# pdishuck/GAVISUNK

Measured on NVIDIA B200. Metric: ont_read_gbp_per_s_sunk_matched_validated, higher is better.
Workload: dtype u64

## Files before the change

### gavisunk_b200/_lib.py

```python
from __future__ import annotations

import ctypes as C
import os

_HERE = os.path.dirname(os.path.abspath(__file__))
LIB_PATH = os.environ.get("GVS_LIB_PATH") or os.path.join(_HERE, "libgavisunk_b200.so")

u8p, u32p, u64p, i32p, i64p, f64p = (C.POINTER(t) for t in (C.c_uint8, C.c_uint32, C.c_uint64, C.c_int32, C.c_int64, C.c_double))
vp = C.c_void_p

PROTOTYPES = {
    "gvs_create": (vp, [C.c_int, C.c_int]),
    "gvs_destroy": (None, [vp]),
    "gvs_last_error": (C.c_char_p, [vp]),
    "gvs_version": (C.c_char_p, []),
    "gvs_set_stream": (C.c_int, [vp, vp]),
    "gvs_sync": (C.c_int, [vp]),
    "gvs_set_profiling": (C.c_int, [vp, C.c_int]),
    "gvs_stage_ms": (C.c_int, [vp, C.c_int, C.POINTER(C.c_float)]),
    "gvs_launch_count": (C.c_uint64, [vp]),
    "gvs_host_alloc": (C.c_int, [C.c_uint64, C.POINTER(vp)]),
    "gvs_host_free": (None, [vp]),
    "gvs_db_load_loc": (C.c_int, [vp, vp, C.c_uint64, vp, vp, vp, vp, C.c_uint64, C.c_uint32]),
    "gvs_db_build": (C.c_int, [vp, vp, vp, C.c_uint32, C.c_int]),
# ... 16 lines not shown
    "gvs_best_get": (C.c_int, [vp, vp, vp, vp, vp]),
    "gvs_filter_best": (C.c_int, [vp, vp, u64p]),
    "gvs_contigs_set": (C.c_int, [vp, vp, vp, C.c_uint32]),
    "gvs_group_hist":(C.c_int, [vp, C.c_int, C.POINTER(vp)]),
    "gvs_hist_mode": (C.c_int, [vp, i64p]),
    "gvs_bad_groups": (C.c_int, [vp, i64p, u64p]),
    "gvs_bad_get": (C.c_int, [vp, vp]),
    "gvs_bad_set": (C.c_int, [vp, vp, vp, C.c_uint64, u64p]),
    "gvs_groups_count": (C.c_int, [vp, u64p]),
    "gvs_groups_get": (C.c_int, [vp, vp, vp, vp]),
    "gvs_batches_begin": (C.c_int, [vp]),
    "gvs_batch_stash": (C.c_int, [vp, u64p]),
    "gvs_batches_bind": (C.c_int, [vp, u64p, u64p]),
    "gvs_validate": (C.c_int, [vp, C.c_uint32, u64p]),
    "gvs_pairs_get": (C.c_int, [vp, vp, vp, vp, vp]),
    "gvs_components_local": (C.c_int, [vp, C.POINTER(vp)]),
    "gvs_components_merge_all": (C.c_int, [vp, vp, C.c_uint32, C.c_uint32]),
    "gvs_placements": (C.c_int, [vp, u64p, C.POINTER(vp)]),
    "gvs_placements_get": (C.c_int, [vp, vp, vp, vp, vp, vp, vp]),
    "gvs_support": (C.c_int, [vp, vp, u64p]),
    "gvs_support_get": (C.c_int, [vp, vp, vp, vp, vp]),
    "gvs_spans": (C.c_int, [vp, C.c_uint32, C.c_uint32, u64p, C.POINTER(vp)]),
    "gvs_spans_get": (C.c_int, [vp] * 9),
    "gvs_discordance": (C.c_int, [vp, vp, u64p]),
    "gvs_discordance_get": (C.c_int, [vp] * 7),
    "gvs_intervals": (C.c_int, [vp, u64p]),
    "gvs_intervals_get": (C.c_int, [vp, vp, vp, vp]),
    "gvs_intervals_set": (C.c_int, [vp, vp, vp, vp, C.c_uint64, C.c_uint32]),
    "gvs_gaps": (C.c_int, [vp, vp, u64p, u64p]),
    "gvs_gaps_get": (C.c_int, [vp, vp, vp, vp, vp]),
# ... 74 lines not shown
```

### gavisunk_b200/csrc/common.cuh

```cuda
#pragma once
#include <cuda_runtime.h>
#include <stdint.h>
#include <stdio.h>
#include <string.h>

#include <string>
#include <vector>

#include "../../include/gavisunk_b200.h"

typedef uint8_t u8;
typedef uint16_t u16;
typedef uint32_t u32;
typedef uint64_t u64;
typedef int32_t i32;
typedef int64_t i64;

#define GVS_NSM_DEFAULT 148
#define GVS_TILE_BASES 512
#define GVS_SEG_COUNT 16
#define GVS_SEG_COUNT_PACK 48
#define GVS_SEG_MIN_BYTES (256ull << 20)

struct DevBuf {
  void* p = nullptr;
  size_t cap = 0;
  template <typename T>
  T* as() const { return (T*)p; }
};

struct Rows {
  DevBuf read, pos, contig, start, group, gidx;
  u64 n = 0;
};

struct RecTable {
  DevBuf buf;
// ... 1 lines not shown
  bool ready = false;
  u32* col(u32 t) const { return buf.as<u32>() + t * stride; }
};

struct gvs_ctx {
  int device = 0;
  int k = 20;
  int n_sm = GVS_NSM_DEFAULT;
  cudaStream_t stream = 0;
  std::string err;
  u64 launches = 0;
  bool profiling = false;
  cudaEvent_t ev0[GVS_ST_COUNT], ev1[GVS_ST_COUNT];
  bool ev_valid[GVS_ST_COUNT];
  std::vector<void*> pinned;
  cudaStream_t aux[2] = {nullptr, nullptr};
  bool val_attr_set = false;
  int l2_persist_max = -1, l2_window_max = 0;
  size_t l2_carve_set = 0;
  cudaEvent_t ev_fork = nullptr, ev_join[2] = {nullptr, nullptr};

  bool db_ready = false;
  u64 n_loc = 0, n_groups = 0;
  u32 n_contigs = 0;
  DevBuf loc_kmer, loc_contig, loc_start, loc_group, loc_gidx;
  DevBuf loc_pack;
  DevBuf grp_contig, grp_start;
  u64 grp_gen = 0;
  DevBuf tab_keys, tab_rows, tab_kv;
  u64 tab_slots = 0;
  DevBuf filt;
  u64 filt_words = 0;
  bool filt_fp = false;
  int probe_variant = 0;
  DevBuf filt1;
// ... 140 lines not shown
                      cudaGetErrorString(e__));                                             \
  } while (0)

#define LAUNCH_ON(strm, kern, grid, block, smem, ...)                                       \
  do {                                                                                      \
    kern<<<(grid), (block), (smem), (strm)>>>(__VA_ARGS__);                                 \
    ctx->launches++;                                                                        \
    cudaError_t e__ = cudaGetLastError();                                                   \
    if (e__ != cudaSuccess)                                                                 \
      return gvs_fail(ctx, GVS_E_CUDA, "%s:%d launch %s: %s", __FILE__, __LINE__, #kern,    \
                      cudaGetErrorString(e__));                                             \
  } while (0)

static inline int gvs_fork(gvs_ctx* ctx) {
  if (!ctx->aux[0]) {
    for (int i = 0; i < 2; i++) {
      CK(cudaStreamCreateWithFlags(&ctx->aux[i], cudaStreamNonBlocking));
      CK(cudaEventCreateWithFlags(&ctx->ev_join[i], cudaEventDisableTiming));
    }
    CK(cudaEventCreateWithFlags(&ctx->ev_fork, cudaEventDisableTiming));
  }
  CK(cudaEventRecord(ctx->ev_fork, ctx->stream));
  for (int i = 0; i < 2; i++) CK(cudaStreamWaitEvent(ctx->aux[i], ctx->ev_fork, 0));
  return 0;
}
static inline int gvs_join(gvs_ctx* ctx) {
  for (int i = 0; i < 2; i++) {
    CK(cudaEventRecord(ctx->ev_join[i], ctx->aux[i]));
    CK(cudaStreamWaitEvent(ctx->stream, ctx->ev_join[i], 0));
  }
  return 0;
}

static inline int gvs_reserve(gvs_ctx* ctx, DevBuf& b, size_t bytes) {
  if (bytes == 0) bytes = 16;
  if (b.cap >= bytes) return 0;
  if (b.p) {
    CK(cudaStreamSynchronize(ctx->stream));
    CK(cudaFree(b.p));
    b.p = nullptr;
    b.cap = 0;
  }
// ... 309 lines not shown
```

### gavisunk_b200/csrc/ctx.cu

```cuda
#include "common.cuh"

#include <sched.h>
#include <stdlib.h>

#include <atomic>
#include <chrono>
#include <condition_variable>
#include <mutex>
#include <thread>

extern "C" void gvs_hostpack_range(const uint8_t* ascii, uint64_t n, uint32_t* words, uint64_t w0, uint64_t w1);

struct HostPipe {
  std::vector<std::thread> workers;
  std::mutex mu;
  std::condition_variable cv_job, cv_done;
  u64 gen = 0;
  bool quit = false;
  int running = 0;
  const u8* ascii = nullptr;
  u64 n = 0;
  u32* words = nullptr;
  u64 w_end = 0;
  std::atomic<u64> next{0};
// ... 145 lines not shown
                   &c->seg_orient, &c->rank_of, &c->rank_grp, &c->sup_diff, &c->pl_strand, &c->pl_tmp,
                   &c->sup_depth, &c->sup_gx, &c->sup_cstat, &c->ge_seg_start, &c->ge_cgap, &c->ge_seg, &c->ge_cand, &c->ge_res,
                   &c->jn_seg_start, &c->jn_row_seg, &c->jn_seg_cnt, &c->jn_flags, &c->jn_scr, &c->dc_diff, &c->dc_scr, &c->dc_seg,
                   &c->pl.buf, &c->sup.buf, &c->ge.buf, &c->jn.buf, &c->dc.buf, &c->dc_runs.buf, &c->rh_scratch, &c->rh.buf,
                   &c->rh_run.buf};
  for (DevBuf* b : all) gvs_release(*b);
  release_rows(c->rows);
  release_rows(c->kept);
  release_rows(c->jn_stash);
  release_rows(c->stash);
  gvs_release(c->stash_len);
  for (int i = 0; i < GVS_ST_COUNT; i++) {
    cudaEventDestroy(c->ev0[i]);
    cudaEventDestroy(c->ev1[i]);
  }
  for (int i = 0; i < 2; i++) {
    if (c->aux[i]) {
      cudaStreamSynchronize(c->aux[i]);
      cudaStreamDestroy(c->aux[i]);
    }
    if (c->ev_join[i]) cudaEventDestroy(c->ev_join[i]);
  }
  if (c->ev_fork) cudaEventDestroy(c->ev_fork);
  for (cudaEvent_t e : c->seg_ev) cudaEventDestroy(e);
  if (c->ev_reads_free) cudaEventDestroy(c->ev_reads_free);
  if (c->copy_stream) {
    cudaStreamSynchronize(c->copy_stream);
    cudaStreamDestroy(c->copy_stream);
  }
  if (c->mailbox) cudaFreeHost(c->mailbox);
  delete c;
// ... 283 lines not shown
```

### gavisunk_b200/csrc/validate_reads.cu

```cuda
#include "common.cuh"

#define VCAP_WARP 64
#define VCAP 512
#define VROW_BYTES 80
#define NOV 0xFFFFFFFFu
#define NOT64 0xFFFFFFFFFFFFFFFFull

#define F_MULTI 1u
#define F_GOOD 2u
#define F_PRES 4u

struct VWork {
  u32 *P, *S, *ID, *G;
  u32 *uP, *uS, *uID, *uG;
  u32 *deg, *rep, *label, *csize, *flags;
  u64 *key, *tv, *ct;
};

__device__ __forceinline__ void vwork_carve(VWork& w, u8* base, u32 cap) {
  u64* q = (u64*)base;
  w.key = q; q += cap;
  w.tv = q; q += cap;
  w.ct = q; q += cap;
  u32* p = (u32*)q;
// ... 3 lines not shown
}

__device__ __forceinline__ bool pair_ok(u32 pi, u32 si, u32 pj, u32 sj) {
  u64 ds = si > sj ? si - sj : sj - si;
  u64 dp = pi > pj ? pi - pj : pj - pi;
  return 9 * ds < 10 * dp && 10 * dp < 11 * ds;
}

struct ValParams : SegRows {
  ReadLens len;
  u32 min_len;
  u32* out_id;
  u32* out_gidx;
  u32* seg_cnt;
  u8* orient;
  u32 m_lo, m_hi;
  u8* gscratch;
  u32 big_cap;
  u32* stats;
};

template <int NT, int GROUPS, bool GLOBAL>
__global__ void __launch_bounds__(NT* GROUPS) k_validate(const ValParams V) {
  extern __shared__ __align__(16) u8 smem[];
  __shared__ u32 s_n0[GROUPS], s_n1[GROUPS], s_m[GROUPS], s_kept[GROUPS], s_bestroot[GROUPS], s_flag[GROUPS], s_dup[GROUPS];
  __shared__ u32 s_pmin[GROUPS], s_pmax[GROUPS];
  __shared__ u32 s_up[GROUPS], s_dn[GROUPS];
  __shared__ unsigned long long s_best[GROUPS];
  __shared__ u32 s_wtot[GROUPS][NT / 32];
  const int grp = threadIdx.x / NT;
  const int tid = threadIdx.x % NT;
  auto gsync = [&]() {
    if (NT == 32) __syncwarp(); else __syncthreads();
  };
  VWork w;
  const u32 cap = GLOBAL ? V.big_cap : (NT == 32 ? VCAP_WARP : VCAP);
  if (GLOBAL) vwork_carve(w, V.gscratch + (u64)blockIdx.x * VROW_BYTES * cap, cap);
  else vwork_carve(w, smem + (u64)grp * VROW_BYTES * cap, cap);

  for (u32 s = blockIdx.x * GROUPS + grp; s < V.n_seg; s += gridDim.x * GROUPS) {
    const u32 a = V.seg_start[s], b = V.seg_start[s + 1];
    const u32 mrows = b - a;
    if (mrows <= V.m_lo || mrows > V.m_hi) continue;
    gsync();
    if (tid == 0) { s_m[grp] = 0; s_n0[grp] = 0; s_n1[grp] = 0; s_kept[grp] = 0; s_best[grp] = 0; s_bestroot[grp] = NOV; s_flag[grp] = 0; s_dup[grp] = 0; s_pmin[grp] = 0xFFFFFFFFu; s_pmax[grp] = 0; s_up[grp] = 0; s_dn[grp] = 0; }
    gsync();
    const u32 rd = V.read[a];
    const u32 rlen = V.len(rd);
    const bool skip = rlen < V.min_len || mrows < 2;
    if (!skip) {
      u32 kept_so_far = 0;
      for (u32 base = 0; base < mrows; base += NT) {
        const u32 i = base + tid;
        bool keep = false;
        u32 gi = 0;
        if (i < mrows) {
          gi = V.gidx[a + i];
          keep = !(V.bad && V.bad[gi]);
        }
        const u32 bal = __ballot_sync(0xFFFFFFFFu, keep);
// ... 50 lines not shown
            u32 sj = w.uS[j], pj = w.uP[j];
            rank += (sj < si) | ((sj == si) & (pj < pi));
          }
        }
        w.P[rank] = pi;
        w.S[rank] = si;
        w.ID[rank] = w.uID[i];
        w.G[rank] = w.uG[i];
        w.csize[i] = 0;
        w.tv[i] = NOT64;
        w.ct[i] = NOT64;
      }
    }
    gsync();
    {
      u32 dupl = 0;
      for (u32 i = tid; i + 1 < m; i += NT) dupl |= w.ID[i] >= w.ID[i + 1];
      if (dupl) s_dup[grp] = 1;
    }
    {
      const u32 id0 = w.ID[0];
      u32 any = 0;
      for (u32 i = tid; i < m; i += NT) any |= w.ID[i] != id0;
      if (any) s_flag[grp] = 1;
    }
    gsync();
    if (!s_flag[grp]) {
      if (tid == 0) V.seg_cnt[s] = 0;
      continue;
    }
    {
      u32 pmin = 0xFFFFFFFFu, pmax = 0;
      for (u32 r = tid; r < m; r += NT) {
// ... 112 lines not shown
        w.flags[r] = present ? F_PRES : 0u;
        w.label[r] = present ? (fp != NOV ? fp : r) : NOV;
        w.tv[r] = present ? tmin : NOT64;
        w.ct[r] = NOT64;
      }
      if (tid == 0) s_kept[grp] = orient ? s_n1[grp] : s_n0[grp];
    } else {
      for (u32 r = tid; r < m; r += NT) {
        if (orient) {
          w.deg[r] = w.label[r];
          w.key[r] = w.ct[r];
        }
        w.ct[r] = NOT64;
      }
      gsync();
      for (u32 r = tid; r < m; r += NT) {
        const u32 id = w.ID[r], dr = w.deg[r];
        const u64 kr = w.key[r];
        u32 first = r, multi = 0, good = dr > 0;
        for (u32 q = 0; q < m; q++) {
          u32 same = (w.ID[q] == id);
          u32 dq = w.deg[q];
          first = (same & (q < first)) ? q : first;
          u32 other = same & (q != r) & (dq > 0);
          multi |= other;
          u32 beats = other & ((dq > dr) | ((dq == dr) & (w.key[q] < kr)));
          good &= beats ^ 1u;
        }
        w.rep[r] = first;
        w.flags[r] = ((multi & (dr > 0)) ? F_MULTI : 0u) | (good ? F_GOOD : 0u);
      }
      gsync();
      {
        u32 nk = 0;
        for (u32 r = tid; r < m; r += NT) {
// ... 33 lines not shown
      continue;
    }
    if (tid == 0) { s_n0[grp] = NOV; s_n1[grp] = 0; }
    gsync();
    for (u32 r = tid; r < m; r += NT)
      if (w.flags[r] & F_PRES) atomicMin(&s_n0[grp], w.label[r]);
    gsync();
    {
      const u32 l0 = s_n0[grp];
      u32 differs = 0;
      for (u32 r = tid; r < m; r += NT) differs |= ((w.flags[r] & F_PRES) != 0) & (w.label[r] != l0);
      if (differs) s_n1[grp] = 1;
    }
    gsync();
    const bool in_row_order = !s_dup[grp] && s_n1[grp] == 0;
    for (int round = 0; s_n1[grp] && round < 4096; round++) {
      if (tid == 0) s_flag[grp] = 0;
      gsync();
      u32 changed = 0;
      for (u32 r = tid; r < m; r += NT) {
        const u32 fr = w.flags[r];
        if (!(fr & F_PRES)) continue;
        const u32 pr = w.P[r], sr = w.S[r], idr = w.ID[r];
        u32 lab = w.label[r];
        const u32 lab0 = lab;
        for (u32 q = 0; q < m; q++) {
          u32 pq = w.P[q], sq = w.S[q], idq = w.ID[q], fq = w.flags[q];
          u32 hi = q > r;
          u32 sg = hi ? (pr > pq) : (pq > pr);
          u32 e = pair_ok(pr, sr, pq, sq) & (q != r) & (sg == orient);
          u32 fl = hi ? fr : fq, fh = hi ? fq : fr;
          u32 drop = ((fl & F_MULTI) != 0) & ((fl & F_GOOD) == 0) & (((fh & F_GOOD) == 0) | (idq != idr));
          u32 link = (e & (drop ^ 1u)) | ((idq == idr) & ((fq & F_PRES) != 0));
          u32 lq = w.label[q];
          lab = (link && lq < lab) ? lq : lab;
        }
        if (lab != lab0) {
          w.label[r] = lab;
          changed = 1;
        }
      }
      if (changed) s_flag[grp] = 1;
      gsync();
      if (!s_flag[grp]) break;
      gsync();
    }
    for (u32 r = tid; r < m; r += NT) {
      u32 fr = w.flags[r];
      if (!(fr & F_PRES)) continue;
      const u32 idr = w.ID[r];
      u32 firstp = r;
      if (s_dup[grp])
        for (u32 q = 0; q < r; q++)
          if (w.ID[q] == idr && (w.flags[q] & F_PRES)) { firstp = q; break; }
      if (firstp != r) continue;
      u32 lab = w.label[r];
      atomicAdd(&w.csize[lab], 1u);
      atomicMin((unsigned long long*)&w.ct[lab], (unsigned long long)w.tv[w.rep[r]]);
      w.flags[r] = fr | 8u;
    }
    gsync();
    for (u32 r = tid; r < m; r += NT) {
      if (w.csize[r]) {
        unsigned long long key = ((unsigned long long)w.csize[r] << 42) | ((1ull << 42) - 1 - w.ct[r]);
        atomicMax(&s_best[grp], key);
      }
    }
    gsync();
// ... 20 lines not shown
          total = 0;
          for (int wv = 0; wv < NT / 32; wv++) {
            const u32 c = s_wtot[grp][wv];
            before += wv < (tid >> 5) ? c : 0u;
            total += c;
          }
        }
        if (mem) {
          const u32 rank = done + before + __popc(bal & ((1u << (tid & 31)) - 1));
          V.out_id[a + rank] = w.ID[r];
          V.out_gidx[a + rank] = w.G[r];
        }
        done += total;
        if (NT > 32) gsync();
      }
    } else
    for (u32 r = tid; r < m; r += NT) {
      if ((w.flags[r] & 8u) && w.label[r] == broot) {
        const u64 t = w.tv[w.rep[r]];
        u32 rank = 0;
        for (u32 q = 0; q < m; q++) rank += ((w.flags[q] & 8u) != 0) & (w.label[q] == broot) & (w.tv[w.rep[q]] < t);
        V.out_id[a + rank] = w.ID[r];
        V.out_gidx[a + rank] = w.G[r];
      }
    }
    if (tid == 0) {
      V.seg_cnt[s] = w.csize[broot];
      V.orient[s] = (u8)orient;
    }
  }
}

__global__ void __launch_bounds__(256) k_pairs_compact(const u32* __restrict__ seg_start, const u32* __restrict__ seg_cnt,
                                                       const u32* __restrict__ seg_off, u32 n_seg, const u32* __restrict__ out_id,
                                                       const u32* __restrict__ out_gidx, const u32* __restrict__ read,
                                                       const u32* __restrict__ contig, u32* p_read, u32* p_contig, u32* p_group,
                                                       u32* p_gidx) {
  u32 wv = (blockIdx.x * blockDim.x + threadIdx.x) >> 5;
  int lane = threadIdx.x & 31;
  if (wv >= n_seg) return;
  u32 c = seg_cnt[wv];
  if (!c) return;
  u32 a = seg_start[wv], o = seg_off[wv];
  u32 rd = read[a], ct = contig[a];
// ... 7 lines not shown

extern "C" int gvs_validate(gvs_ctx* ctx, uint32_t min_read_len, uint64_t* n_pairs_out) {
  if (!ctx) return GVS_E_ARG;
  if (!ctx->diag_ready) return gvs_fail(ctx, GVS_E_STATE, "gvs_validate before gvs_diag_filter / gvs_rows_set(1)");
  if (!ctx->read_off && !ctx->have_read_len) return gvs_fail(ctx, GVS_E_STATE, "gvs_validate: read lengths unknown");
  CK(cudaSetDevice(ctx->device));
  StageTimer tm(ctx, GVS_ST_VALIDATE);
  ctx->val_ready = false;
  ctx->pl.ready = ctx->sup.ready = false;
  ctx->dc.ready = ctx->dc_runs.ready = false;
  ctx->n_pairs = 0;
  if (n_pairs_out) *n_pairs_out = 0;
  Rows& R = ctx->kept;
  u64 n = R.n;
  if (n == 0) {
    ctx->val_ready = true;
    return 0;
  }
  u64 n_seg = 0;
  CKR(gvs_build_segments(ctx, R.read.as<u32>(), n, ctx->kseg_start, ctx->flags_c, &n_seg));
  ctx->n_kseg = n_seg;
  const u32* seg_start = ctx->kseg_start.as<u32>();
  CKR(gvs_reserve(ctx, ctx->val_scratch, (2 * n + 2 * n_seg + 16) * 4));
  u32* out_id = ctx->val_scratch.as<u32>();
  u32* out_gidx = out_id + n;
  u32* seg_cnt = out_gidx + n;
  u32* seg_off = seg_cnt + n_seg;
  ctx->val_id = out_id; ctx->val_seg_cnt = seg_cnt; ctx->val_seg_off = seg_off;
  CKR(gvs_reserve(ctx, ctx->seg_orient, n_seg));
  u32 max_m = 0;
  {
    auto f2 = [seg_start] __device__(u64 s) -> u32 { return seg_start[s + 1] - seg_start[s]; };
    auto g2 = [] __device__(u64 s, u32 ex, u32 v) {};
    CKR(scan_total(ctx, n_seg, f2, g2, OpMax(), &max_m));
  }
  u32* stats = counter(ctx, CNT_VAL_STATS);
  CK(cudaMemsetAsync(stats, 0, 8, ctx->stream));
  ValParams V;
  (SegRows&)V = seg_rows(ctx, R, ctx->kseg_start, n_seg);
  V.len = read_lens(ctx);
  V.min_len = min_read_len;
  V.out_id = out_id; V.out_gidx = out_gidx; V.seg_cnt = seg_cnt; V.orient = ctx->seg_orient.as<u8>();
  V.gscratch = nullptr; V.big_cap = 0; V.stats = stats;
  const size_t sm_warp = (size_t)VROW_BYTES * VCAP_WARP * 8, sm_blk = (size_t)VROW_BYTES * VCAP;
  if (!ctx->val_attr_set) {
    CK(cudaFuncSetAttribute((k_validate<32, 8, false>), cudaFuncAttributeMaxDynamicSharedMemorySize, (int)sm_warp));
    CK(cudaFuncSetAttribute((k_validate<256, 1, false>), cudaFuncAttributeMaxDynamicSharedMemorySize, (int)sm_blk));
    ctx->val_attr_set = true;
  }
  const bool tiers = max_m > VCAP_WARP;
  if (tiers) CKR(gvs_fork(ctx));
  if (max_m > VCAP) {
    u32 blocks = (u32)ctx->n_sm;
    u32 bcap = (max_m + 15) & ~15u;
    CKR(gvs_reserve(ctx, ctx->scan_tmp2, (u64)blocks * VROW_BYTES * bcap));
    V.gscratch = ctx->scan_tmp2.as<u8>();
    V.big_cap = bcap;
    V.m_lo = VCAP; V.m_hi = 0xFFFFFFFFu;
    LAUNCH_ON(ctx->aux[1], (k_validate<1024, 1, true>), blocks, 1024, 0, V);
    V.gscratch = nullptr; V.big_cap = 0;
  }
  if (max_m > VCAP_WARP) {
    V.m_lo = VCAP_WARP; V.m_hi = VCAP;
    u64 grid = n_seg;
    u64 capg = (u64)ctx->n_sm * 5;
    if (grid > capg) grid = capg;
    LAUNCH_ON(ctx->aux[0], (k_validate<256, 1, false>), (unsigned)grid, 256, sm_blk, V);
  }
  {
    V.m_lo = 0; V.m_hi = VCAP_WARP;
    u64 grid = cdiv(n_seg, 8);
    u64 capg = (u64)ctx->n_sm * 5;
    if (grid > capg) grid = capg;
    LAUNCH((k_validate<32, 8, false>), (unsigned)grid, 256, sm_warp, V);
  }
  if (tiers) CKR(gvs_join(ctx));
  u32 np = 0;
  {
    auto f = [seg_cnt] __device__(u64 s) -> u32 { return seg_cnt[s]; };
    auto g = [seg_off] __device__(u64 s, u32 ex, u32 v) { seg_off[s] = ex; };
    CKR(scan_total(ctx, n_seg, f, g, OpSum(), &np));
  }
  CKR(gvs_reserve(ctx, ctx->pair_read, (u64)np * 4));
  CKR(gvs_reserve(ctx, ctx->pair_contig, (u64)np * 4));
  CKR(gvs_reserve(ctx, ctx->pair_group, (u64)np * 4));
  CKR(gvs_reserve(ctx, ctx->pair_gidx, (u64)np * 4));
  if (np)
    LAUNCH(k_pairs_compact, (unsigned)cdiv(n_seg * 32, 256), 256, 0, seg_start, seg_cnt, seg_off, (u32)n_seg, out_id, out_gidx,
           R.read.as<u32>(), R.contig.as<u32>(), ctx->pair_read.as<u32>(), ctx->pair_contig.as<u32>(),
           ctx->pair_group.as<u32>(), ctx->pair_gidx.as<u32>());
  ctx->n_pairs = np;
  ctx->val_ready = true;
  if (n_pairs_out) *n_pairs_out = np;
  return 0;
}

extern "C" int gvs_pairs_get(gvs_ctx* ctx, uint32_t* read_idx, uint32_t* contig, uint32_t* group, uint32_t* group_index) {
  if (!ctx) return GVS_E_ARG;
  if (!ctx->val_ready) return gvs_fail(ctx, GVS_E_STATE, "gvs_pairs_get before gvs_validate");
  CK(cudaSetDevice(ctx->device));
  u64 n = ctx->n_pairs;
  if (n == 0) return 0;
  if (read_idx) CK(cudaMemcpyAsync(read_idx, ctx->pair_read.p, n * 4, cudaMemcpyDeviceToHost, ctx->stream));
  if (contig) CK(cudaMemcpyAsync(contig, ctx->pair_contig.p, n * 4, cudaMemcpyDeviceToHost, ctx->stream));
  if (group) CK(cudaMemcpyAsync(group, ctx->pair_group.p, n * 4, cudaMemcpyDeviceToHost, ctx->stream));
  if (group_index) CK(cudaMemcpyAsync(group_index, ctx->pair_gidx.p, n * 4, cudaMemcpyDeviceToHost, ctx->stream));
  CK(cudaStreamSynchronize(ctx->stream));
  return 0;
}
```

### gavisunk_b200/engine.py

```python
from __future__ import annotations

import ctypes as C
import math
from typing import Dict, List, Optional, Sequence, Tuple

import numpy as np

from . import _lib
from ._lib import GavisunkError, GavisunkKeyError

GVS_HAP_ANY = 2

_LUT = np.zeros(256, dtype=np.uint64)
for _ch, _v in (("A", 0), ("C", 1), ("G", 2), ("T", 3), ("U", 3)):
    _LUT[ord(_ch)] = _v
    _LUT[ord(_ch.lower())] = _v
_LUT[1], _LUT[2], _LUT[3] = 1, 2, 3


def encode_kmers(lines: Sequence[bytes], k: Optional[int] = None) -> np.ndarray:
    if len(lines) == 0:
        return np.zeros(0, dtype=np.uint64)
    if k is None:
        k = len(lines[0])
# ... 418 lines not shown
        self.n_bad = int(n.value)
        return self.n_bad

    def groups(self, with_hist: bool = False) -> Dict[str, np.ndarray]:
        n = C.c_uint64()
        self._ck(self.lib.gvs_groups_count(self.ctx, C.byref(n)))
        return self._table("groups", self.lib.gvs_groups_get, int(n.value), ("contig", "group", "count" if with_hist else None),
                           dtypes=dict(count=np.int32))

    def validate(self, min_read_len: int = 10000) -> int:
        n = C.c_uint64()
        self._ck(self.lib.gvs_validate(self.ctx, min_read_len, C.byref(n)))
        self.n_pairs = int(n.value)
        return self.n_pairs

    PAIR_COLUMNS = ("read", "contig", "group", "gidx")

    def pairs(self, pinned: bool = False) -> Dict[str, np.ndarray]:
        return self._table("pairs", self.lib.gvs_pairs_get, self.n_pairs, self.PAIR_COLUMNS, pinned=pinned)

    PLACEMENT_COLUMNS = ("read", "contig", "start", "end", "n_ids", "strand")

    def placements(self, pinned: bool = False) -> Dict[str, np.ndarray]:
        n, p = C.c_uint64(), C.c_void_p()
        self._ck(self.lib.gvs_placements(self.ctx, C.byref(n), C.byref(p)))
        self._diff_ptr = int(p.value or 0)
        return self._table("placements", self.lib.gvs_placements_get, int(n.value), self.PLACEMENT_COLUMNS,
                           dtypes=dict(strand=np.uint8), pinned=pinned)

    SUPPORT_COLUMNS = ("contig", "start", "end", "depth")
# ... 148 lines not shown
```

### include/gavisunk_b200.h

```cpp
#ifndef GAVISUNK_B200_H
#define GAVISUNK_B200_H

#include <stdint.h>

#ifdef __cplusplus
extern "C" {
#endif

typedef struct gvs_ctx gvs_ctx;

enum {
  GVS_OK = 0,
  GVS_E_CUDA = -1,
  GVS_E_ARG = -2,
  GVS_E_KEYERROR = -3,
  GVS_E_NOMEM = -4,
  GVS_E_OVERFLOW = -5,
  GVS_E_STATE = -6
};

enum {
  GVS_ST_PROBE = 0,
  GVS_ST_EMIT = 1,
  GVS_ST_DIAG = 2,
// ... 116 lines not shown
int gvs_group_hist(gvs_ctx* ctx, int accumulate, int32_t** hist_dev);
int gvs_hist_mode(gvs_ctx* ctx, int64_t mode[2]);
int gvs_bad_groups(gvs_ctx* ctx, const int64_t limit_floor[2], uint64_t* n_bad);
int gvs_bad_get(gvs_ctx* ctx, uint32_t* group_index );
int gvs_bad_set(gvs_ctx* ctx, const uint32_t* contig, const uint32_t* group, uint64_t n, uint64_t* n_bad);
int gvs_groups_count(gvs_ctx* ctx, uint64_t* n_groups);
int gvs_groups_get(gvs_ctx* ctx, uint32_t* contig, uint32_t* group, int32_t* hist);

int gvs_batches_begin(gvs_ctx* ctx);
int gvs_batch_stash(gvs_ctx* ctx, uint64_t* read_base);
int gvs_batches_bind(gvs_ctx* ctx, uint64_t* n_rows, uint64_t* n_reads);

int gvs_validate(gvs_ctx* ctx, uint32_t min_read_len, uint64_t* n_pairs);
int gvs_pairs_get(gvs_ctx* ctx, uint32_t* read_idx, uint32_t* contig, uint32_t* group,
                  uint32_t* group_index);

int gvs_components_local(gvs_ctx* ctx, uint32_t** parent_dev);
int gvs_components_merge_all(gvs_ctx* ctx, const uint32_t* gathered_dev, uint32_t n_ranks, uint32_t own_rank);
int gvs_intervals(gvs_ctx* ctx, uint64_t* n_intervals);
int gvs_intervals_get(gvs_ctx* ctx, uint32_t* contig, uint32_t* start, uint32_t* end);

int gvs_placements(gvs_ctx* ctx, uint64_t* n, int32_t** diff_dev);
int gvs_placements_get(gvs_ctx* ctx, uint32_t* read_idx, uint32_t* contig, uint32_t* start, uint32_t* end, uint32_t* n_ids,
                       uint8_t* strand);
int gvs_support(gvs_ctx* ctx, const uint32_t* contig_len, uint64_t* n_runs);
int gvs_support_get(gvs_ctx* ctx, uint32_t* contig, uint32_t* start, uint32_t* end, uint32_t* depth);

int gvs_spans(gvs_ctx* ctx, uint32_t min_delta, uint32_t rel_permille, uint64_t* n_records, int32_t** diff_dev);
int gvs_spans_get(gvs_ctx* ctx, uint32_t* read, uint32_t* contig, uint32_t* id1, uint32_t* start1, uint32_t* pos1, uint32_t* id2,
                  uint32_t* start2, uint32_t* pos2);
// ... 45 lines not shown
```

Before: 395.6.

## Bucket validate segments into size tiers and use union-find labeling

Adds a classification kernel that puts each read segment into one of four size tiers. A new 128-thread mid tier runs on a third aux stream, and each kernel walks only its own compacted segment list, so blocks no longer scan and skip out-of-range segments. The iterative min-label propagation is replaced with a single-pass atomic union-find. The O(m^2) duplicate-ID scan is narrowed to the equal-ID neighbourhood when IDs are sorted, and rank-by-counting output ordering becomes a bitonic sort. Grids are now sized from occupancy queries. The risks are extra launches, a host readback of tier counts, and atomic contention in union-find.

```diff
diff --git a/gavisunk_b200/_lib.py b/gavisunk_b200/_lib.py
--- a/gavisunk_b200/_lib.py
+++ b/gavisunk_b200/_lib.py
@@ -54,6 +54,7 @@
     "gvs_batches_bind": (C.c_int, [vp, u64p, u64p]),
     "gvs_validate": (C.c_int, [vp, C.c_uint32, u64p]),
     "gvs_pairs_get": (C.c_int, [vp, vp, vp, vp, vp]),
+    "gvs_validate_stats": (C.c_int, [vp, C.POINTER(C.c_uint32), C.POINTER(C.c_uint32)]),
     "gvs_components_local": (C.c_int, [vp, C.POINTER(vp)]),
     "gvs_components_merge_all": (C.c_int, [vp, vp, C.c_uint32, C.c_uint32]),
     "gvs_placements": (C.c_int, [vp, u64p, C.POINTER(vp)]),
diff --git a/gavisunk_b200/csrc/common.cuh b/gavisunk_b200/csrc/common.cuh
--- a/gavisunk_b200/csrc/common.cuh
+++ b/gavisunk_b200/csrc/common.cuh
@@ -21,6 +21,7 @@
 #define GVS_SEG_COUNT 16
 #define GVS_SEG_COUNT_PACK 48
 #define GVS_SEG_MIN_BYTES (256ull << 20)
+#define GVS_N_AUX 3
 
 struct DevBuf {
   void* p = nullptr;
@@ -52,11 +53,12 @@
   cudaEvent_t ev0[GVS_ST_COUNT], ev1[GVS_ST_COUNT];
   bool ev_valid[GVS_ST_COUNT];
   std::vector<void*> pinned;
-  cudaStream_t aux[2] = {nullptr, nullptr};
+  cudaStream_t aux[GVS_N_AUX] = {};
   bool val_attr_set = false;
+  int val_resident[3] = {};
   int l2_persist_max = -1, l2_window_max = 0;
   size_t l2_carve_set = 0;
-  cudaEvent_t ev_fork = nullptr, ev_join[2] = {nullptr, nullptr};
+  cudaEvent_t ev_fork = nullptr, ev_join[GVS_N_AUX] = {};
 
   bool db_ready = false;
   u64 n_loc = 0, n_groups = 0;
@@ -227,18 +229,18 @@
 
 static inline int gvs_fork(gvs_ctx* ctx) {
   if (!ctx->aux[0]) {
-    for (int i = 0; i < 2; i++) {
+    for (int i = 0; i < GVS_N_AUX; i++) {
       CK(cudaStreamCreateWithFlags(&ctx->aux[i], cudaStreamNonBlocking));
       CK(cudaEventCreateWithFlags(&ctx->ev_join[i], cudaEventDisableTiming));
     }
     CK(cudaEventCreateWithFlags(&ctx->ev_fork, cudaEventDisableTiming));
   }
   CK(cudaEventRecord(ctx->ev_fork, ctx->stream));
-  for (int i = 0; i < 2; i++) CK(cudaStreamWaitEvent(ctx->aux[i], ctx->ev_fork, 0));
+  for (int i = 0; i < GVS_N_AUX; i++) CK(cudaStreamWaitEvent(ctx->aux[i], ctx->ev_fork, 0));
   return 0;
 }
 static inline int gvs_join(gvs_ctx* ctx) {
-  for (int i = 0; i < 2; i++) {
+  for (int i = 0; i < GVS_N_AUX; i++) {
     CK(cudaEventRecord(ctx->ev_join[i], ctx->aux[i]));
     CK(cudaStreamWaitEvent(ctx->stream, ctx->ev_join[i], 0));
   }
diff --git a/gavisunk_b200/csrc/ctx.cu b/gavisunk_b200/csrc/ctx.cu
--- a/gavisunk_b200/csrc/ctx.cu
+++ b/gavisunk_b200/csrc/ctx.cu
@@ -183,7 +183,7 @@
     cudaEventDestroy(c->ev0[i]);
     cudaEventDestroy(c->ev1[i]);
   }
-  for (int i = 0; i < 2; i++) {
+  for (int i = 0; i < GVS_N_AUX; i++) {
     if (c->aux[i]) {
       cudaStreamSynchronize(c->aux[i]);
       cudaStreamDestroy(c->aux[i]);
diff --git a/gavisunk_b200/csrc/validate_reads.cu b/gavisunk_b200/csrc/validate_reads.cu
--- a/gavisunk_b200/csrc/validate_reads.cu
+++ b/gavisunk_b200/csrc/validate_reads.cu
@@ -1,6 +1,7 @@
 #include "common.cuh"
 
 #define VCAP_WARP 64
+#define VCAP_MID 256
 #define VCAP 512
 #define VROW_BYTES 80
 #define NOV 0xFFFFFFFFu
@@ -41,16 +42,19 @@
   u32* out_gidx;
   u32* seg_cnt;
   u8* orient;
-  u32 m_lo, m_hi;
+  const u32* list;
+  const u32* list_n;
   u8* gscratch;
   u32 big_cap;
   u32* stats;
 };
 
-template <int NT, int GROUPS, bool GLOBAL>
+template <int NT, int GROUPS, int CAP, bool GLOBAL>
 __global__ void __launch_bounds__(NT* GROUPS) k_validate(const ValParams V) {
+  static_assert(GLOBAL || (CAP & (CAP - 1)) == 0, "capacity must be a power of two");
   extern __shared__ __align__(16) u8 smem[];
   __shared__ u32 s_n0[GROUPS], s_n1[GROUPS], s_m[GROUPS], s_kept[GROUPS], s_bestroot[GROUPS], s_flag[GROUPS], s_dup[GROUPS];
+  __shared__ u32 s_unsorted[GROUPS];
   __shared__ u32 s_pmin[GROUPS], s_pmax[GROUPS];
   __shared__ u32 s_up[GROUPS], s_dn[GROUPS];
   __shared__ unsigned long long s_best[GROUPS];
@@ -61,16 +65,17 @@
     if (NT == 32) __syncwarp(); else __syncthreads();
   };
   VWork w;
-  const u32 cap = GLOBAL ? V.big_cap : (NT == 32 ? VCAP_WARP : VCAP);
+  const u32 cap = GLOBAL ? V.big_cap : CAP;
   if (GLOBAL) vwork_carve(w, V.gscratch + (u64)blockIdx.x * VROW_BYTES * cap, cap);
   else vwork_carve(w, smem + (u64)grp * VROW_BYTES * cap, cap);
 
-  for (u32 s = blockIdx.x * GROUPS + grp; s < V.n_seg; s += gridDim.x * GROUPS) {
+  const u32 n_list = *V.list_n;
+  for (u32 li = blockIdx.x * GROUPS + grp; li < n_list; li += gridDim.x * GROUPS) {
+    const u32 s = V.list[li];
     const u32 a = V.seg_start[s], b = V.seg_start[s + 1];
     const u32 mrows = b - a;
-    if (mrows <= V.m_lo || mrows > V.m_hi) continue;
-    gsync();
-    if (tid == 0) { s_m[grp] = 0; s_n0[grp] = 0; s_n1[grp] = 0; s_kept[grp] = 0; s_best[grp] = 0; s_bestroot[grp] = NOV; s_flag[grp] = 0; s_dup[grp] = 0; s_pmin[grp] = 0xFFFFFFFFu; s_pmax[grp] = 0; s_up[grp] = 0; s_dn[grp] = 0; }
+    gsync();
+    if (tid == 0) { s_m[grp] = 0; s_n0[grp] = 0; s_n1[grp] = 0; s_kept[grp] = 0; s_best[grp] = 0; s_bestroot[grp] = NOV; s_flag[grp] = 0; s_dup[grp] = 0; s_unsorted[grp] = 0; s_pmin[grp] = 0xFFFFFFFFu; s_pmax[grp] = 0; s_up[grp] = 0; s_dn[grp] = 0; }
     gsync();
     const u32 rd = V.read[a];
     const u32 rlen = V.len(rd);
@@ -151,9 +156,13 @@
     }
     gsync();
     {
-      u32 dupl = 0;
-      for (u32 i = tid; i + 1 < m; i += NT) dupl |= w.ID[i] >= w.ID[i + 1];
+      u32 dupl = 0, unsorted = 0;
+      for (u32 i = tid; i + 1 < m; i += NT) {
+        dupl |= w.ID[i] >= w.ID[i + 1];
+        unsorted |= w.ID[i] > w.ID[i + 1];
+      }
       if (dupl) s_dup[grp] = 1;
+      if (unsorted) s_unsorted[grp] = 1;
     }
     {
       const u32 id0 = w.ID[0];
@@ -296,11 +305,19 @@
         w.ct[r] = NOT64;
       }
       gsync();
+      const bool ids_sorted = !s_unsorted[grp];
       for (u32 r = tid; r < m; r += NT) {
         const u32 id = w.ID[r], dr = w.deg[r];
         const u64 kr = w.key[r];
         u32 first = r, multi = 0, good = dr > 0;
-        for (u32 q = 0; q < m; q++) {
+        u32 qlo = 0, qhi = m;
+        if (ids_sorted) {
+          qlo = r;
+          qhi = r + 1;
+          while (qlo > 0 && w.ID[qlo - 1] == id) qlo--;
+          while (qhi < m && w.ID[qhi] == id) qhi++;
+        }
+        for (u32 q = qlo; q < qhi; q++) {
           u32 same = (w.ID[q] == id);
           u32 dq = w.deg[q];
           first = (same & (q < first)) ? q : first;
@@ -364,35 +381,57 @@
     }
     gsync();
     const bool in_row_order = !s_dup[grp] && s_n1[grp] == 0;
-    for (int round = 0; s_n1[grp] && round < 4096; round++) {
-      if (tid == 0) s_flag[grp] = 0;
-      gsync();
-      u32 changed = 0;
+    if (tid == 0 && s_n1[grp]) atomicAdd(&V.stats[1], 1u);
+    if (s_n1[grp]) {
+      volatile u32* par = w.uP;
+      for (u32 r = tid; r < m; r += NT) par[r] = r;
+      gsync();
+      auto find = [&](u32 x) -> u32 {
+        u32 cur = par[x];
+        if (cur != x) {
+          u32 nxt, prev = x;
+          while (cur > (nxt = par[cur])) {
+            par[prev] = nxt;
+            prev = cur;
+            cur = nxt;
+          }
+        }
+        return cur;
+      };
+      auto unite = [&](u32 x, u32 y) {
+        u32 rx = find(x), ry = find(y);
+        while (rx != ry) {
+          if (rx < ry) {
+            const u32 old = atomicCAS((u32*)&par[ry], ry, rx);
+            if (old == ry) break;
+            ry = old;
+          } else {
+            const u32 old = atomicCAS((u32*)&par[rx], rx, ry);
+            if (old == rx) break;
+            rx = old;
+          }
+        }
+      };
       for (u32 r = tid; r < m; r += NT) {
         const u32 fr = w.flags[r];
         if (!(fr & F_PRES)) continue;
         const u32 pr = w.P[r], sr = w.S[r], idr = w.ID[r];
-        u32 lab = w.label[r];
-        const u32 lab0 = lab;
-        for (u32 q = 0; q < m; q++) {
-          u32 pq = w.P[q], sq = w.S[q], idq = w.ID[q], fq = w.flags[q];
-          u32 hi = q > r;
-          u32 sg = hi ? (pr > pq) : (pq > pr);
-          u32 e = pair_ok(pr, sr, pq, sq) & (q != r) & (sg == orient);
-          u32 fl = hi ? fr : fq, fh = hi ? fq : fr;
-          u32 drop = ((fl & F_MULTI) != 0) & ((fl & F_GOOD) == 0) & (((fh & F_GOOD) == 0) | (idq != idr));
-          u32 link = (e & (drop ^ 1u)) | ((idq == idr) & ((fq & F_PRES) != 0));
-          u32 lq = w.label[q];
-          lab = (link && lq < lab) ? lq : lab;
-        }
-        if (lab != lab0) {
-          w.label[r] = lab;
-          changed = 1;
-        }
-      }
-      if (changed) s_flag[grp] = 1;
-      gsync();
-      if (!s_flag[grp]) break;
+        if (w.rep[r] != r) unite(r, w.rep[r]);
+        for (u32 q = r + 1; q < m; q++) {
+          const u32 pq = w.P[q], sq = w.S[q], idq = w.ID[q], fq = w.flags[q];
+          const u32 e = pair_ok(pr, sr, pq, sq) & ((pr > pq) == orient);
+          const u32 drop = ((fr & F_MULTI) != 0) & ((fr & F_GOOD) == 0) & (((fq & F_GOOD) == 0) | (idq != idr));
+          const u32 link = (e & (drop ^ 1u)) | ((idq == idr) & ((fq & F_PRES) != 0));
+          if (link) unite(r, q);
+        }
+      }
+      gsync();
+      for (u32 r = tid; r < m; r += NT)
+        if (w.flags[r] & F_PRES) {
+          u32 x = r;
+          while (par[x] != x) x = par[x];
+          w.label[r] = x;
+        }
       gsync();
     }
     for (u32 r = tid; r < m; r += NT) {
@@ -401,7 +440,7 @@
       const u32 idr = w.ID[r];
       u32 firstp = r;
       if (s_dup[grp])
-        for (u32 q = 0; q < r; q++)
+        for (u32 q = w.rep[r]; q < r; q++)
           if (w.ID[q] == idr && (w.flags[q] & F_PRES)) { firstp = q; break; }
       if (firstp != r) continue;
       u32 lab = w.label[r];
@@ -452,20 +491,73 @@
         done += total;
         if (NT > 32) gsync();
       }
-    } else
-    for (u32 r = tid; r < m; r += NT) {
-      if ((w.flags[r] & 8u) && w.label[r] == broot) {
-        const u64 t = w.tv[w.rep[r]];
-        u32 rank = 0;
-        for (u32 q = 0; q < m; q++) rank += ((w.flags[q] & 8u) != 0) & (w.label[q] == broot) & (w.tv[w.rep[q]] < t);
-        V.out_id[a + rank] = w.ID[r];
-        V.out_gidx[a + rank] = w.G[r];
+    } else {
+      u64* sk = w.key;
+      u32* sv = w.deg;
+      if (tid == 0) s_n0[grp] = 0;
+      gsync();
+      for (u32 r = tid; r < m; r += NT)
+        if ((w.flags[r] & 8u) && w.label[r] == broot) {
+          const u32 slot = atomicAdd(&s_n0[grp], 1u);
+          sk[slot] = w.tv[w.rep[r]];
+          sv[slot] = r;
+        }
+      gsync();
+      const u32 k = s_n0[grp];
+      u32 n2 = 1;
+      while (n2 < k) n2 <<= 1;
+      for (u32 i = k + tid; i < n2; i += NT) sk[i] = NOT64;
+      gsync();
+      for (u32 len = 2; len <= n2; len <<= 1)
+        for (u32 j = len >> 1; j; j >>= 1) {
+          for (u32 i = tid; i < n2; i += NT) {
+            const u32 ij = i ^ j;
+            if (ij > i) {
+              const u64 ki = sk[i], kj = sk[ij];
+              if ((ki > kj) == ((i & len) == 0)) {
+                sk[i] = kj;
+                sk[ij] = ki;
+                const u32 t = sv[i];
+                sv[i] = sv[ij];
+                sv[ij] = t;
+              }
+            }
+          }
+          gsync();
+        }
+      for (u32 i = tid; i < k; i += NT) {
+        const u32 r = sv[i];
+        V.out_id[a + i] = w.ID[r];
+        V.out_gidx[a + i] = w.G[r];
       }
     }
     if (tid == 0) {
       V.seg_cnt[s] = w.csize[broot];
       V.orient[s] = (u8)orient;
     }
+  }
+}
+
+__global__ void __launch_bounds__(256) k_val_tiers(const u32* __restrict__ seg_start, u32 n_seg, u32* list, u32* cnt) {
+  const u32 s = blockIdx.x * blockDim.x + threadIdx.x;
+  const int lane = threadIdx.x & 31;
+  u32 m = 0;
+  int t = -1;
+  if (s < n_seg) {
+    m = seg_start[s + 1] - seg_start[s];
+    t = m <= VCAP_WARP ? 0 : m <= VCAP_MID ? 1 : m <= VCAP ? 2 : 3;
+  }
+  u32 mx = m;
+  for (int d = 16; d; d >>= 1) mx = max(mx, __shfl_xor_sync(0xFFFFFFFFu, mx, d));
+  if (lane == 0 && mx) atomicMax(&cnt[4], mx);
+  for (int k = 0; k < 4; k++) {
+    const u32 bal = __ballot_sync(0xFFFFFFFFu, t == k);
+    if (!bal) continue;
+    const int leader = __ffs(bal) - 1;
+    u32 base = 0;
+    if (lane == leader) base = atomicAdd(&cnt[k], (u32)__popc(bal));
+    base = __shfl_sync(0xFFFFFFFFu, base, leader);
+    if (t == k) list[(u64)k * n_seg + base + __popc(bal & ((1u << lane) - 1))] = s;
   }
 }
 
@@ -503,6 +595,7 @@
   Rows& R = ctx->kept;
   u64 n = R.n;
   if (n == 0) {
+    ctx->n_kseg = 0;
     ctx->val_ready = true;
     return 0;
   }
@@ -510,19 +603,20 @@
   CKR(gvs_build_segments(ctx, R.read.as<u32>(), n, ctx->kseg_start, ctx->flags_c, &n_seg));
   ctx->n_kseg = n_seg;
   const u32* seg_start = ctx->kseg_start.as<u32>();
-  CKR(gvs_reserve(ctx, ctx->val_scratch, (2 * n + 2 * n_seg + 16) * 4));
+  CKR(gvs_reserve(ctx, ctx->val_scratch, (2 * n + 6 * n_seg + 16) * 4));
   u32* out_id = ctx->val_scratch.as<u32>();
   u32* out_gidx = out_id + n;
   u32* seg_cnt = out_gidx + n;
   u32* seg_off = seg_cnt + n_seg;
+  u32* tier_list = seg_off + n_seg;
+  u32* tier_cnt = tier_list + 4 * n_seg;
   ctx->val_id = out_id; ctx->val_seg_cnt = seg_cnt; ctx->val_seg_off = seg_off;
   CKR(gvs_reserve(ctx, ctx->seg_orient, n_seg));
-  u32 max_m = 0;
-  {
-    auto f2 = [seg_start] __device__(u64 s) -> u32 { return seg_start[s + 1] - seg_start[s]; };
-    auto g2 = [] __device__(u64 s, u32 ex, u32 v) {};
-    CKR(scan_total(ctx, n_seg, f2, g2, OpMax(), &max_m));
-  }
+  u32 tc[5];
+  CK(cudaMemsetAsync(tier_cnt, 0, 8 * 4, ctx->stream));
+  LAUNCH(k_val_tiers, (unsigned)cdiv(n_seg, 256), 256, 0, seg_start, (u32)n_seg, tier_list, tier_cnt);
+  CKR(read_dev(ctx, tier_cnt, tc, 5));
+  const u32 max_m = tc[4];
   u32* stats = counter(ctx, CNT_VAL_STATS);
   CK(cudaMemsetAsync(stats, 0, 8, ctx->stream));
   ValParams V;
@@ -531,37 +625,50 @@
   V.min_len = min_read_len;
   V.out_id = out_id; V.out_gidx = out_gidx; V.seg_cnt = seg_cnt; V.orient = ctx->seg_orient.as<u8>();
   V.gscratch = nullptr; V.big_cap = 0; V.stats = stats;
-  const size_t sm_warp = (size_t)VROW_BYTES * VCAP_WARP * 8, sm_blk = (size_t)VROW_BYTES * VCAP;
+  const size_t sm_warp = (size_t)VROW_BYTES * VCAP_WARP * 8, sm_mid = (size_t)VROW_BYTES * VCAP_MID,
+               sm_blk = (size_t)VROW_BYTES * VCAP;
   if (!ctx->val_attr_set) {
-    CK(cudaFuncSetAttribute((k_validate<32, 8, false>), cudaFuncAttributeMaxDynamicSharedMemorySize, (int)sm_warp));
-    CK(cudaFuncSetAttribute((k_validate<256, 1, false>), cudaFuncAttributeMaxDynamicSharedMemorySize, (int)sm_blk));
+    CK(cudaFuncSetAttribute((k_validate<32, 8, VCAP_WARP, false>), cudaFuncAttributeMaxDynamicSharedMemorySize, (int)sm_warp));
+    CK(cudaFuncSetAttribute((k_validate<128, 1, VCAP_MID, false>), cudaFuncAttributeMaxDynamicSharedMemorySize, (int)sm_mid));
+    CK(cudaFuncSetAttribute((k_validate<256, 1, VCAP, false>), cudaFuncAttributeMaxDynamicSharedMemorySize, (int)sm_blk));
+    CK(cudaOccupancyMaxActiveBlocksPerMultiprocessor(&ctx->val_resident[0], k_validate<32, 8, VCAP_WARP, false>, 256, sm_warp));
+    CK(cudaOccupancyMaxActiveBlocksPerMultiprocessor(&ctx->val_resident[1], k_validate<128, 1, VCAP_MID, false>, 128, sm_mid));
+    CK(cudaOccupancyMaxActiveBlocksPerMultiprocessor(&ctx->val_resident[2], k_validate<256, 1, VCAP, false>, 256, sm_blk));
+    for (int i = 0; i < 3; i++) ctx->val_resident[i] = ctx->val_resident[i] > 0 ? ctx->val_resident[i] : 1;
     ctx->val_attr_set = true;
   }
-  const bool tiers = max_m > VCAP_WARP;
+  auto grid_of = [&](u64 blocks, int tier) -> unsigned {
+    const u64 capg = (u64)ctx->n_sm * ctx->val_resident[tier];
+    return (unsigned)(blocks < capg ? blocks : capg);
+  };
+  const bool tiers = tc[1] + tc[2] + tc[3] > 0;
   if (tiers) CKR(gvs_fork(ctx));
-  if (max_m > VCAP) {
-    u32 blocks = (u32)ctx->n_sm;
-    u32 bcap = (max_m + 15) & ~15u;
+  auto use_tier = [&](int t) {
+    V.list = tier_list + (u64)t * n_seg;
+    V.list_n = tier_cnt + t;
+  };
+  if (tc[3]) {
+    u32 blocks = min((u32)ctx->n_sm, tc[3]);
+    u32 bcap = 16;
+    while (bcap < max_m) bcap <<= 1;
     CKR(gvs_reserve(ctx, ctx->scan_tmp2, (u64)blocks * VROW_BYTES * bcap));
     V.gscratch = ctx->scan_tmp2.as<u8>();
     V.big_cap = bcap;
-    V.m_lo = VCAP; V.m_hi = 0xFFFFFFFFu;
-    LAUNCH_ON(ctx->aux[1], (k_validate<1024, 1, true>), blocks, 1024, 0, V);
+    use_tier(3);
+    LAUNCH_ON(ctx->aux[2], (k_validate<1024, 1, 0, true>), blocks, 1024, 0, V);
     V.gscratch = nullptr; V.big_cap = 0;
   }
-  if (max_m > VCAP_WARP) {
-    V.m_lo = VCAP_WARP; V.m_hi = VCAP;
-    u64 grid = n_seg;
-    u64 capg = (u64)ctx->n_sm * 5;
-    if (grid > capg) grid = capg;
-    LAUNCH_ON(ctx->aux[0], (k_validate<256, 1, false>), (unsigned)grid, 256, sm_blk, V);
-  }
-  {
-    V.m_lo = 0; V.m_hi = VCAP_WARP;
-    u64 grid = cdiv(n_seg, 8);
-    u64 capg = (u64)ctx->n_sm * 5;
-    if (grid > capg) grid = capg;
-    LAUNCH((k_validate<32, 8, false>), (unsigned)grid, 256, sm_warp, V);
+  if (tc[2]) {
+    use_tier(2);
+    LAUNCH_ON(ctx->aux[1], (k_validate<256, 1, VCAP, false>), grid_of(tc[2], 2), 256, sm_blk, V);
+  }
+  if (tc[1]) {
+    use_tier(1);
+    LAUNCH_ON(ctx->aux[0], (k_validate<128, 1, VCAP_MID, false>), grid_of(tc[1], 1), 128, sm_mid, V);
+  }
+  if (tc[0]) {
+    use_tier(0);
+    LAUNCH((k_validate<32, 8, VCAP_WARP, false>), grid_of(cdiv(tc[0], 8), 0), 256, sm_warp, V);
   }
   if (tiers) CKR(gvs_join(ctx));
   u32 np = 0;
@@ -584,6 +691,17 @@
   return 0;
 }
 
+extern "C" int gvs_validate_stats(gvs_ctx* ctx, uint32_t* empty_reads, uint32_t* searched_reads) {
+  if (!ctx) return GVS_E_ARG;
+  if (!ctx->val_ready) return gvs_fail(ctx, GVS_E_STATE, "gvs_validate_stats before gvs_validate");
+  CK(cudaSetDevice(ctx->device));
+  u32 st[2] = {0, 0};
+  if (ctx->n_kseg) CKR(read_dev(ctx, counter(ctx, CNT_VAL_STATS), st, 2));
+  if (empty_reads) *empty_reads = st[0];
+  if (searched_reads) *searched_reads = st[1];
+  return 0;
+}
+
 extern "C" int gvs_pairs_get(gvs_ctx* ctx, uint32_t* read_idx, uint32_t* contig, uint32_t* group, uint32_t* group_index) {
   if (!ctx) return GVS_E_ARG;
   if (!ctx->val_ready) return gvs_fail(ctx, GVS_E_STATE, "gvs_pairs_get before gvs_validate");
diff --git a/gavisunk_b200/engine.py b/gavisunk_b200/engine.py
--- a/gavisunk_b200/engine.py
+++ b/gavisunk_b200/engine.py
@@ -456,6 +456,11 @@
         self.n_pairs = int(n.value)
         return self.n_pairs
 
+    def validate_stats(self) -> Tuple[int, int]:
+        a, b = C.c_uint32(), C.c_uint32()
+        self._ck(self.lib.gvs_validate_stats(self.ctx, C.byref(a), C.byref(b)))
+        return int(a.value), int(b.value)
+
     PAIR_COLUMNS = ("read", "contig", "group", "gidx")
 
     def pairs(self, pinned: bool = False) -> Dict[str, np.ndarray]:
diff --git a/include/gavisunk_b200.h b/include/gavisunk_b200.h
--- a/include/gavisunk_b200.h
+++ b/include/gavisunk_b200.h
@@ -154,6 +154,7 @@
 int gvs_validate(gvs_ctx* ctx, uint32_t min_read_len, uint64_t* n_pairs);
 int gvs_pairs_get(gvs_ctx* ctx, uint32_t* read_idx, uint32_t* contig, uint32_t* group,
                   uint32_t* group_index);
+int gvs_validate_stats(gvs_ctx* ctx, uint32_t* empty_reads, uint32_t* searched_reads);
 
 int gvs_components_local(gvs_ctx* ctx, uint32_t** parent_dev);
 int gvs_components_merge_all(gvs_ctx* ctx, const uint32_t* gathered_dev, uint32_t n_ranks, uint32_t own_rank);
diff --git a/profiles/validate_stage.py b/profiles/validate_stage.py
--- /dev/null
+++ b/profiles/validate_stage.py
@@ -0,0 +1,141 @@
+import argparse
+import hashlib
+import json
+import os
+import subprocess
+import sys
+
+import numpy as np
+
+ROOT = os.path.dirname(os.path.dirname(os.path.abspath(__file__)))
+sys.path.insert(0, ROOT)
+
+TIERS = [("warp", 0, 64), ("blk128", 64, 256), ("blk256", 256, 512), ("global", 512, 1 << 32)]
+
+
+def gpu_info():
+    try:
+        out = subprocess.run(["nvidia-smi", "--query-gpu=name,power.limit,clocks.max.sm", "--format=csv,noheader", "-i", "0"],
+                             capture_output=True, text=True, timeout=20).stdout.strip()
+    except Exception as ex:
+        out = f"nvidia-smi unavailable: {ex}"
+    return out
+
+
+def classify(kept, grp_contig, grp_start, bad, read_len, min_len=10000):
+    read = kept["read"].astype(np.int64)
+    n = len(read)
+    gkey = (grp_contig.astype(np.uint64) << np.uint64(32)) | grp_start.astype(np.uint64)
+    order = np.argsort(gkey, kind="stable")
+    rkey = (kept["contig"].astype(np.uint64) << np.uint64(32)) | kept["group"].astype(np.uint64)
+    gidx = order[np.searchsorted(gkey[order], rkey)]
+    assert np.array_equal(gkey[gidx], rkey)
+    is_bad = np.zeros(len(gkey), bool)
+    is_bad[bad] = True
+    brk = np.flatnonzero(np.diff(read)) + 1
+    seg_a = np.concatenate([[0], brk])
+    seg_b = np.concatenate([brk, [n]])
+    mrows = seg_b - seg_a
+    seg_of_row = np.repeat(np.arange(len(seg_a)), mrows)
+    keep = ~is_bad[gidx]
+    m = np.bincount(seg_of_row[keep], minlength=len(seg_a))
+    active = (read_len[read[seg_a]] >= min_len) & (mrows >= 2) & (m >= 2)
+    sel = keep & active[seg_of_row]
+    s, p, g, sg = kept["start"][sel], kept["pos"][sel], kept["group"][sel], seg_of_row[sel]
+    o = np.lexsort((p, s, sg))
+    s, p, g, sg = s[o], p[o], g[o], sg[o]
+    same = sg[1:] == sg[:-1]
+    nseg = len(seg_a)
+
+    def any_by_seg(flag):
+        return np.bincount(sg[1:][same & flag], minlength=nseg) > 0
+    dup = any_by_seg(g[:-1] >= g[1:])
+    multi_group = any_by_seg(g[:-1] != g[1:])
+    up = any_by_seg(p[:-1] < p[1:])
+    dn = any_by_seg(p[:-1] > p[1:])
+    tested = active & multi_group
+    path = np.full(nseg, "skipped", dtype=object)
+    path[tested & ~dup & ~(up & dn)] = "fast"
+    path[tested & ~dup & up & dn] = "nonmono"
+    path[tested & dup] = "dup"
+    out = {}
+    for name, lo, hi in TIERS:
+        t = (mrows > lo) & (mrows <= hi)
+        row = {}
+        for pth in ("skipped", "fast", "nonmono", "dup"):
+            k = t & (path == pth)
+            row[pth] = dict(reads=int(k.sum()), rows=int(mrows[k].sum()), rows_sq=int((mrows[k].astype(np.int64) ** 2).sum()))
+        out[name] = row
+    return out
+
+
+def tier_of_kernel(name):
+    if "k_validate<32," in name:
+        return "warp"
+    if "k_validate<128," in name:
+        return "blk128"
+    if "k_validate<256," in name:
+        return "blk256"
+    if "k_validate<1024," in name:
+        return "global"
+    return None
+
+
+def main():
+    ap = argparse.ArgumentParser()
+    ap.add_argument("--reps", type=int, default=30)
+    ap.add_argument("--warmup", type=int, default=3)
+    a = ap.parse_args()
+    import torch
+    from gavisunk_b200 import workload as W
+    from gavisunk_b200.engine import Engine
+    if not torch.cuda.is_available():
+        raise SystemExit("validate_stage.py measures on a GPU; none found")
+    eng = Engine(20)
+    contigs = W.human_contigs(3100.0)
+    wl = W.make_assembly(eng, contigs, snp_rate=1e-3, dup_frac=0.01, seed=1001, name="h3100")
+    W.build_db(eng, wl)
+    batch_args = dict(coverage=3.75, n50=100000.0, sigma=0.8, len_min=1000, len_max=1000000, nchunks=10)
+    batches = [W.new_batch(eng, wl, seed=2001 + 16 * b, **batch_args) for b in range(8)]
+    binds = [(lambda e, b=b: W.bind_batch(e, b)) for b in batches]
+    eng.set_profiling(True)
+    eng.run_batches(binds, wl.contig_hap, min_read_len=10000)
+    stage = []
+    for i in range(a.warmup + a.reps):
+        eng.validate(10000)
+        if i >= a.warmup:
+            stage.append(eng.stage_ms("validate"))
+    stage = np.array(stage)
+    try:
+        n_empty, n_searched = eng.validate_stats()
+    except AttributeError:
+        n_empty = n_searched = None
+    pr = eng.pairs()
+    digest = hashlib.sha256(b"".join(np.ascontiguousarray(pr[c]).tobytes() for c in eng.PAIR_COLUMNS)).hexdigest()[:16]
+    from torch.profiler import ProfilerActivity, profile
+    with profile(activities=[ProfilerActivity.CUDA]) as prof:
+        for _ in range(a.reps):
+            eng.validate(10000)
+        eng.sync()
+    per = {}
+    for e in prof.events():
+        t = tier_of_kernel(e.name)
+        if t is not None:
+            per.setdefault(t, []).append(e.time_range.elapsed_us() / 1000.0)
+    tier_ms = {t: dict(median=float(np.median(v)), min=float(np.min(v)), max=float(np.max(v)), launches=len(v))
+               for t, v in per.items()}
+    kept = eng.rows(1)
+    g = eng.groups()
+    lens = np.concatenate([np.diff(b.read_off.cpu().numpy()) for b in batches]).astype(np.int64)
+    census = classify(kept, g["contig"], g["group"], eng.bad_list().astype(np.int64), lens)
+    print(json.dumps(dict(
+        metric="validate_stage_ms", workload="h3100 (bench.py default: 3.1 Gbp x2, 8 batches of 3.75x, k 20), 1 GPU",
+        gpu=gpu_info(), reps=a.reps, kept_rows=int(eng.n_kept), reads=int(eng.n_reads), validated_pairs=int(eng.n_pairs),
+        pairs_digest=digest, validate_ms_median=float(np.median(stage)), validate_ms_min=float(stage.min()),
+        validate_ms_max=float(stage.max()), tier_ms=tier_ms, empty_reads=n_empty, searched_reads=n_searched,
+        census=census)))
+    eng.close()
+
+
+if __name__ == "__main__":
+    main()
```

Result: no change. 399.5, median of 6 (+1.0%).
